# wyhuai/DDNM

Measured on AMD Instinct MI355X. Metric: restored images/sec @256×256, 100 DDIM steps, 4×SR; 1/2/4/8 GPU, higher is better.
Workload: dtype f32 (3x3 convolutions: fp32 operands carried as hi + lo fp16 halves, three fp16 MFMA products per product, fp32 accumulate -- operand error 2^-22, measured closer to fp64 than the fp32 MFMA kernel; everything else fp32); 1 GPU; celeba_hq.yml SVD sr_bicubic 4x, sigma_y=0, eta=0.85, T_sampling=100, batch_size=8 per GPU (BASELINE configs[1]); global_batch=8, image=3x256x256, parallelism=dp1 (image sharding)

## Files before the change

ddnm_amd/_lib.py:

```python
import ctypes
import os
from ctypes import POINTER, Structure, c_char_p, c_float, c_int32, c_int64, c_uint8, c_uint32, c_void_p

_HERE = os.path.dirname(os.path.abspath(__file__))
LIB_PATH = os.path.join(_HERE, "libddnm_hip.so")

c_f32p = c_void_p


class ConvDesc(Structure):
    _fields_ = [
        ("src0", c_void_p), ("src1", c_void_p), ("weight", c_void_p), ("bias", c_void_p),
        ("badd", c_void_p), ("res", c_void_p), ("gn_scale", c_void_p), ("gn_shift", c_void_p),
        ("out", c_void_p),
        ("B", c_int32), ("Hin", c_int32), ("Win", c_int32),
        ("C0", c_int32), ("C1", c_int32), ("Cout", c_int32),
        ("ksize", c_int32), ("stride", c_int32), ("pad", c_int32),
        ("Ho", c_int32), ("Wo", c_int32),
        ("ups", c_int32), ("gn_silu", c_int32), ("out_nchw", c_int32),
        ("badd_stride", c_int32), ("tile", c_int32),
        ("workspace", c_void_p), ("workspace_floats", c_int64),
        ("res_ups", c_int32), ("src_f16", c_int32),
        ("stats_out", c_void_p),
        ("skip0", c_void_p), ("skip1", c_void_p), ("skip_weight", c_void_p),
# ... 61 lines not shown
    "ddnm_hq_project_f32": (c_int32, [c_void_p, c_void_p, c_void_p, c_void_p, c_int64, c_float, c_void_p]),
    "ddnm_copy_rect_f32": (c_int32, [c_void_p, c_int32, c_int32, c_int32, c_int32, c_void_p, c_int32, c_int32, c_int32,
                                     c_int32, c_int32, c_int32, c_int32, c_void_p]),
    "ddnm_hq_sample_f32": (c_int32, [c_void_p, c_void_p, c_void_p, c_void_p, c_void_p, c_int64, c_float, c_float, c_float,
                                     c_float, c_void_p]),
    "ddnm_patchify_f32": (c_int32, [c_void_p, c_void_p, c_int32, c_int32, c_int32, c_int32, c_void_p]),
    "ddnm_im2col3x3_f16": (c_int32, [c_void_p, c_void_p, c_void_p, c_void_p, c_void_p, c_int32, c_int32, c_int32, c_int32,
                                     c_int32, c_int32, c_void_p]),
    "ddnm_gn_apply_f16": (c_int32, [c_void_p, c_void_p, c_void_p, c_void_p, c_void_p, c_int32, c_int32, c_int32, c_int32,
                                    c_int32, c_void_p]),
    "ddnm_gn_finalize_tiles_f32": (c_int32, [c_void_p, c_int32, c_int32, c_void_p, c_int32, c_int32, c_void_p, c_void_p,
                                             c_int32, c_int32, c_int32, c_float, c_void_p, c_void_p, c_void_p, c_int32,
                                             c_void_p, c_void_p]),
    "ddnm_gn_finalize_tiles_amax_f32": (c_int32, [c_void_p, c_int32, c_int32, c_void_p, c_int32, c_int32, c_void_p, c_void_p,
                                                  c_int32, c_int32, c_int32, c_float, c_void_p, c_void_p, c_void_p, c_int32,
                                                  c_void_p, c_void_p, c_void_p]),
    "ddnm_amax_bound_f32": (c_int32, [c_void_p, c_int64, c_int32, c_void_p, c_int64, c_int32, c_void_p, c_int32, c_void_p]),
    "ddnm_conv3x3_f16_f32": (c_int32, [POINTER(ConvDesc), c_void_p]),
    "ddnm_conv3x3_f16_supported": (c_int32, [POINTER(ConvDesc)]),
    "ddnm_conv3x3_f16_workspace_floats": (c_int64, [POINTER(ConvDesc)]),
    "ddnm_conv3x3_f16_stats_tiles": (c_int32, [POINTER(ConvDesc)]),
    "ddnm_conv3x3_s16_f32": (c_int32, [POINTER(ConvDesc), c_void_p]),
    "ddnm_conv3x3_s16_supported": (c_int32, [POINTER(ConvDesc)]),
    "ddnm_conv3x3_s16_persistent": (c_int32, [POINTER(ConvDesc)]),
    "ddnm_conv3x3_s16_ups_subpixel_supported": (c_int32, [POINTER(ConvDesc)]),
    "ddnm_conv3x3_s16_workspace_floats": (c_int64, [POINTER(ConvDesc)]),
    "ddnm_conv3x3_s16_stats_tiles": (c_int32, [POINTER(ConvDesc)]),
    "ddnm_conv3x3_s16_act_scale": (c_float, []),
    "ddnm_conv_gather_s16_f32": (c_int32, [POINTER(ConvDesc), c_void_p]),
    "ddnm_conv_gather_s16_supported": (c_int32, [POINTER(ConvDesc)]),
    "ddnm_conv_gather_s16_workspace_floats": (c_int64, [POINTER(ConvDesc)]),
    "ddnm_conv_gather_s16_stats_tiles": (c_int32, [POINTER(ConvDesc)]),
    "ddnm_conv_gather_s16_gemm1x1": (c_int32, [POINTER(ConvDesc)]),
    "ddnm_conv16": (c_int32, [POINTER(Conv16Desc), c_void_p]),
    "ddnm_conv16_supported": (c_int32, [POINTER(Conv16Desc)]),
    "ddnm_conv16_fuses_fin": (c_int32, [POINTER(Conv16Desc)]),
    "ddnm_conv16_workspace_floats": (c_int64, [POINTER(Conv16Desc)]),
    "ddnm_conv16_stats_tiles": (c_int32, [POINTER(Conv16Desc)]),
    "ddnm_gn_apply_h16": (c_int32, [c_void_p, c_void_p, c_void_p, c_void_p, c_void_p, c_int32, c_int32, c_int32, c_int32,
                                    c_int32, c_int32, c_int32, c_void_p]),
    "ddnm_im2col3x3_h16": (c_int32, [c_void_p, c_void_p, c_void_p, c_void_p, c_void_p, c_int32, c_int32, c_int32, c_int32,
                                     c_int32, c_int32, c_void_p]),
    "ddnm_nchw_to_nhwc_h16": (c_int32, [c_void_p, c_void_p, c_int32, c_int32, c_int32, c_int32, c_void_p]),
    "ddnm_gn_stats_h16": (c_int32, [c_void_p, c_void_p, c_int32, c_int32, c_int32, c_int32, c_void_p]),
    "ddnm_attn16_d64": (c_int32, [c_void_p, c_void_p, c_int32, c_int32, c_int32, c_void_p]),
    "ddnm_conv1x1_f16_f32": (c_int32, [POINTER(ConvDesc), c_void_p]),
    "ddnm_conv1x1_f16_supported": (c_int32, [POINTER(ConvDesc)]),
    "ddnm_conv1x1_f16_workspace_floats": (c_int64, [POINTER(ConvDesc)]),
    "ddnm_conv1x1_f16_stats_tiles": (c_int32, [POINTER(ConvDesc)]),
    "ddnm_gn_stats_f32": (c_int32, [c_void_p, c_void_p, c_int32, c_int32, c_int32, c_int32, c_int32, c_void_p,
                                    c_int32, c_void_p]),
    "ddnm_gn_nchunk": (c_int32, [c_int32, c_int32]),
    "ddnm_gn_finalize_f32": (c_int32, [c_void_p, c_int32, c_void_p, c_void_p, c_int32, c_int32, c_int32, c_int32,
                                       c_float, c_void_p, c_void_p, c_void_p, c_int32, c_void_p, c_void_p]),
    "ddnm_bgemm_f32": (c_int32, [POINTER(GemmDesc), c_void_p]),
    "ddnm_gn_bwd_f32": (c_int32, [c_void_p, c_void_p, c_int32, c_void_p, c_void_p, c_void_p, c_int32, c_void_p, c_int32,
                                  c_int32, c_int32, c_int32, c_int32, c_int32, c_void_p, c_int32, c_void_p, c_void_p,
                                  c_void_p]),
    "ddnm_gn_bwd_nchunk": (c_int32, [c_int32, c_int32]),
    "ddnm_gn_bwd_h16": (c_int32, [c_void_p, c_void_p, c_int32, c_void_p, c_void_p, c_void_p, c_int32, c_void_p, c_int32,
                                  c_int32, c_int32, c_int32, c_int32, c_int32, c_void_p, c_int32, c_void_p, c_void_p,
                                  c_void_p]),
    "ddnm_pool_tokens_h16": (c_int32, [c_void_p, c_void_p, c_void_p, c_void_p, c_void_p, c_int32, c_int32, c_int32,
                                       c_void_p]),
    "ddnm_pool_tokens_bwd_h16": (c_int32, [c_void_p, c_void_p, c_int32, c_int32, c_int32, c_void_p]),
    "ddnm_attn16_d64_lse": (c_int32, [c_void_p, c_void_p, c_void_p, c_int32, c_int32, c_int32, c_void_p]),
# ... 165 lines not shown
```

ddnm_amd/build.py:

```python
import hashlib
import os
import shutil
import subprocess
import sys

HERE = os.path.dirname(os.path.abspath(__file__))
CSRC = os.path.join(HERE, "csrc")
LIB = os.path.join(HERE, "libddnm_hip.so")
STAMP = os.path.join(HERE, ".libddnm_hip.stamp")
OBJ = os.path.join(HERE, "_obj")
SOURCES = ["conv_igemm_f32.hip", "conv_igemm_f16.hip", "conv_s16_persist.hip", "conv_s16_subpixel.hip", "conv_gather_s16.hip", "conv1x1_s16.hip", "conv_small_f32.hip", "conv1x1_f16.hip", "conv16.hip", "act16.hip", "attn16.hip", "attn_d512.hip", "attn16_bwd.hip", "gemm_f32.hip", "groupnorm.hip", "misc.hip", "ddnm_step.hip", "fwht.hip", "backward.hip", "metrics.hip"]
FLAGS = ["--offload-arch=gfx950", "-O3", "-std=c++17", "-fPIC", "-shared", "-Wall", "-Wno-unused-function"]


def _hipcc():
    for c in (os.environ.get("HIPCC"), shutil.which("hipcc"), "/opt/rocm/bin/hipcc"):
        if c and os.path.exists(c):
            return c
    raise RuntimeError("hipcc not found (set HIPCC)")


def _digest():
    h = hashlib.sha256()
    for f in sorted(os.listdir(CSRC)) + ["../../include/ddnm_hip.h"]:
        with open(os.path.join(CSRC, f), "rb") as fh:
            h.update(f.encode() + fh.read())
    h.update(" ".join(FLAGS).encode())
    return h.hexdigest()


LAST_BUILD = {"compiled": False}


def build(force=False, verbose=False):
    dig = _digest()
    LAST_BUILD["compiled"] = False
    if not force and os.path.exists(LIB) and os.path.exists(STAMP) and open(STAMP).read() == dig:
        return LIB
    LAST_BUILD["compiled"] = True
    tmp = LIB + f".tmp{os.getpid()}"
    os.makedirs(OBJ, exist_ok=True)
    hh = hashlib.sha256()
    for f in sorted(os.listdir(CSRC)) + ["../../include/ddnm_hip.h"]:
        if f.endswith(".h"):
# ... 54 lines not shown
```

ddnm_amd/csrc/conv1x1_s16.hip:

```cpp
#include "s16_tile.h"

constexpr int G1_KS = 2;
constexpr int G1_BM = 64, G1_BN = 64;
constexpr int G1_AR = G1_BM / 32;
constexpr int G1_BR = G1_BN / 32;
constexpr int G1_NWG = 3;
constexpr int G1_WSUB = G1_BN * 128;
constexpr int G1_ASUB = G1_BM * S16_LDH;
constexpr int G1_REQ_A = G1_KS * (G1_AR + 2);
constexpr int G1_REQ_W = G1_KS * G1_BR;
constexpr int G1_WAIT = 3 * G1_REQ_A + 2 * G1_REQ_W;
constexpr int G1_MAX_CIN = 1024;
constexpr int G1_ROUTE_MAX_CIN = 512;
static_assert(G1_WAIT < 64, "vmcnt counts to 63");

__device__ __forceinline__ void g1_tile_stats(float p0, float p1, float p2, float p3, int rows, float& s, float& q) {
#pragma clang fp contract(off)
    if (rows >= 4) {
        s = ((p0 + p1) + p2) + p3;
        q = ((p0 * p0 + p1 * p1) + p2 * p2) + p3 * p3;
    } else if (rows == 3) {
        s = ((p0 + p3) + p1) + p2;
        q = (__builtin_fmaf(p3, p3, p0 * p0) + p1 * p1) + p2 * p2;
    } else if (rows == 2) {
        s = (p0 + p2) + (p1 + p3);
        q = __builtin_fmaf(p2, p2, p0 * p0) + __builtin_fmaf(p3, p3, p1 * p1);
    } else {
        s = ((p0 + p1) + p2) + p3;
        q = __builtin_fmaf(p3, p3, __builtin_fmaf(p2, p2, __builtin_fmaf(p1, p1, p0 * p0)));
    }
}

__global__ __launch_bounds__(256) void conv1x1_s16_kernel(const ConvArgs p, const int stats_px) {
    __shared__ __attribute__((aligned(1024))) char lds_all[G1_NWG * G1_KS * G1_WSUB + G1_KS * G1_ASUB * 2];
    char* const Bs = lds_all;
    _Float16* const As = reinterpret_cast<_Float16*>(lds_all + G1_NWG * G1_KS * G1_WSUB);

    const ddnm_conv_desc& d = p.d;
    const int tid = threadIdx.x, lane = tid & 63, wave = tid >> 6;
    const int wm = wave >> 1, wn = wave & 1;
    const int tile_id = xcd_swizzle(blockIdx.x, gridDim.x);
    const int n_tile = tile_id % p.n_tiles, m_tile = tile_id / p.n_tiles;
    const int hw = d.Ho * d.Wo;
    const int img = m_tile / (hw / G1_BM);
    const unsigned pix0 = (unsigned)m_tile * G1_BM;
    float ascale, inv_ascale;
    s16_operand_scale(d.gn_scale == nullptr ? d.amax_in : nullptr, img, false, ascale, inv_ascale);

    const int lrow = lane >> 3, lpiece = lane & 7;
    const int wswz = S16_W_SWZ(wave, lrow);
    const unsigned w_rowlen = (unsigned)p.Cin * 4u;
    const int cout_pad = (d.Cout + 127) / 128 * 128;
    const __amdgpu_buffer_rsrc_t r_w = __builtin_amdgcn_make_buffer_rsrc(
        const_cast<void*>(reinterpret_cast<const void*>(d.weight)), 0, (unsigned)cout_pad * w_rowlen, 0x00020000);
    const unsigned w_voff = S16_W_LANE(n_tile * G1_BN + wave * 8 + lrow, w_rowlen, lpiece, wswz);
    const int nchunks = p.Cin / S16_KCH;
    const int nsteps = (nchunks + G1_KS - 1) / G1_KS;
    auto chunk_of = [&](int s, int sub) { const int c = s * G1_KS + sub; return c < nchunks ? c : nchunks - 1; };
    auto issue_w = [&](int s, int grp) {
#pragma unroll
        for (int sub = 0; sub < G1_KS; ++sub)
            s16_w_request<G1_BR, 4>(r_w, Bs + (grp * G1_KS + sub) * G1_WSUB + wave * 1024, w_voff, (unsigned)chunk_of(s, sub) * S16_KCH * 4u,
                                    w_rowlen);
    };
// ... 127 lines not shown
    }
    if (ksplit == 1) {
        float add = 0.f;
        if (d.bias) add = bias;
        if (d.badd) add += badd;
#pragma unroll
        for (int r = 0; r < 16; ++r) v[r] = acc[0][0][r] * epi + add + rv[r];
    } else if (d.stats_out) {
        float add = 0.f;
        if (d.bias) add = add + bias;
        if (d.badd) add = add + badd;
#pragma unroll
        for (int r = 0; r < 16; ++r) {
            v[r] = add + total[r] * epi;
            if (res) v[r] = v[r] + rv[r];
        }
    } else {
#pragma unroll
        for (int r = 0; r < 16; ++r) {
            v[r] = total[r] * epi;
            if (d.bias) v[r] = v[r] + bias;
            if (d.badd) v[r] = v[r] + badd;
            if (res) v[r] = v[r] + rv[r];
        }
    }
#pragma unroll
    for (int r = 0; r < 16; ++r) out[o[r]] = v[r];
    if (stats_px == 4) {
        const unsigned t0 = (pix0 + wm * 32 + rsel) >> 2;
        const int rows = 256 / (d.Cout >> 2);
#pragma unroll
        for (int q = 0; q < 4; ++q) {
            float cs, cq;
            g1_tile_stats(v[q * 4], v[q * 4 + 1], v[q * 4 + 2], v[q * 4 + 3], rows, cs, cq);
            float2* const st = reinterpret_cast<float2*>(d.stats_out + ((size_t)(t0 + 2 * q) * d.Cout + n) * 2);
            *st = make_float2(cs, cq);
        }
    } else if (stats_px == G1_BM) {
        float cs = 0.f, cq = 0.f;
#pragma unroll
        for (int r = 0; r < 16; ++r) {
            cs += v[r];
            cq = __builtin_fmaf(v[r], v[r], cq);
        }
        cs += __shfl_xor(cs, 32);
        cq += __shfl_xor(cq, 32);
        float* const lds = reinterpret_cast<float*>(As);
        __syncthreads();
        if (lane < 32) {
            lds[(wm * G1_BN + wn * 32 + lane) * 2 + 0] = cs;
            lds[(wm * G1_BN + wn * 32 + lane) * 2 + 1] = cq;
        }
        __syncthreads();
        if (tid < G1_BN * 2) {
            const int c = tid >> 1, which = tid & 1;
            d.stats_out[((size_t)m_tile * d.Cout + n_tile * G1_BN + c) * 2 + which] = lds[c * 2 + which] + lds[(G1_BN + c) * 2 + which];
        }
    }
}

int conv1x1_s16_stats_px(const ddnm_conv_desc* d, int plan_ksplit, int plan_bm) {
    if (!d->stats_out) return 0;
    if (plan_ksplit > 1) {
        const int tpi = splitk_stats_tiles(d);
        return tpi > 0 && d->Ho * d->Wo == 4 * tpi ? 4 : -1;
    }
    return plan_bm == G1_BM ? G1_BM : -1;
}

bool conv1x1_s16_routes(const ddnm_conv_desc* d, int plan_ksplit, int plan_bm) {
    const int hw = d->Ho * d->Wo, Cin = d->C0 + d->C1;
    if (d->ksize != 1 || d->stride != 1 || d->pad != 0 || d->ups || d->res_ups || d->out_nchw || d->skip0) return false;
    if (d->Ho != d->Hin || d->Wo != d->Win || hw % G1_BM || d->Cout % G1_BN) return false;
    if (d->C0 <= 0 || d->C0 % S16_KCH || d->C1 % S16_KCH || Cin > G1_MAX_CIN) return false;
    if (conv1x1_s16_stats_px(d, plan_ksplit, plan_bm) < 0) return false;
    if (d->flags & DDNM_CONV_GEMM1X1) return true;
    return Cin <= G1_ROUTE_MAX_CIN;
}

int conv1x1_s16_launch(const ddnm_conv_desc* d, int plan_ksplit, int plan_bm, int run_ksplit, hipStream_t s) {
    const ConvArgs p = conv_args(*d, G1_BM, d->Cout / G1_BN, 32, 5, 0, 1, run_ksplit);
    DDNM_LAUNCH(conv1x1_s16_kernel, dim3(p.m_tiles * p.n_tiles), dim3(256), 0, s, p, conv1x1_s16_stats_px(d, plan_ksplit, plan_bm));
    return 0;
}
```

ddnm_amd/csrc/conv_common.h:

```cpp
#pragma once
#include "common.h"

struct ConvArgs {
    ddnm_conv_desc d;
    int Cin, ntaps, Hs, Ws;
    int m_tiles, n_tiles;
    int tiles_x;
    int TW, TW_log2;
    int ksplit;
    float* ws;
};

static inline bool conv_operand_offsets_fit(const ddnm_conv_desc* d) {
    const int64_t px = (int64_t)d->B * (d->ups ? d->Hin / 2 : d->Hin) * (d->ups ? d->Win / 2 : d->Win);
    const int64_t cmax = d->C0 > d->C1 ? d->C0 : d->C1;
    return px * cmax * (d->src_f16 ? 2 : 4) < (int64_t)1 << 31;
}
static inline bool conv_sizes_addressable(const ddnm_conv_desc* d) {
    const int64_t lim = (int64_t)1 << 31;
    const int64_t out_el = (int64_t)d->B * d->Ho * d->Wo * d->Cout;
    const int64_t cout_pad = ((int64_t)d->Cout + 127) / 128 * 128;
    const int64_t w_b = cout_pad * d->ksize * d->ksize * ((int64_t)d->C0 + d->C1) * 4;
    const int64_t sk_el = (int64_t)d->B * d->Ho * d->Wo * (d->SC0 > d->SC1 ? d->SC0 : d->SC1);
    return out_el < lim && conv_operand_offsets_fit(d) && w_b < lim && sk_el < lim;
}

bool conv3x3_s16_persist_eligible(const ConvArgs& p);
int conv3x3_s16_persist_launch(const ConvArgs& p, hipStream_t s);
bool conv3x3_s16_ups_subpixel_ok(const ddnm_conv_desc* d);
int conv3x3_s16_ups_subpixel_run(const ddnm_conv_desc* d, hipStream_t s);
bool conv1x1_s16_routes(const ddnm_conv_desc* d, int plan_ksplit, int plan_bm);
int conv1x1_s16_launch(const ddnm_conv_desc* d, int plan_ksplit, int plan_bm, int run_ksplit, hipStream_t s);
int conv_persist_grid_cus();

struct TileMap {
    int img, ty0, tx0, th_unused, TW, TW_log2, flat_base, Wo;
    bool two_d;
    __device__ __forceinline__ void pixel(int r, int& oy, int& ox) const {
        if (two_d) {
            oy = ty0 + (r >> TW_log2);
            ox = tx0 + (r & (TW - 1));
        } else {
            const int pix = flat_base + r;
            oy = pix / Wo;
            ox = pix - oy * Wo;
        }
    }
};

template <int BM>
__device__ __forceinline__ TileMap make_tilemap(const ConvArgs& p, int m_tile) {
    TileMap t;
    const int HWo = p.d.Ho * p.d.Wo;
    const int per_img = HWo / BM;
    t.img = m_tile / per_img;
    const int t_in_img = m_tile - t.img * per_img;
    t.TW = p.TW;
    t.TW_log2 = p.TW_log2;
    t.Wo = p.d.Wo;
    t.two_d = p.tiles_x != 0;
    if (t.two_d) {
        const int ty = t_in_img / p.tiles_x, tx = t_in_img - ty * p.tiles_x;
        t.ty0 = ty * (BM >> p.TW_log2);
        t.tx0 = tx << p.TW_log2;
        t.flat_base = 0;
// ... 236 lines not shown
            if (d.res) {
                if (d.res_ups) {
                    const int oy = p2 / d.Wo, ox = p2 - oy * d.Wo;
                    v = v + *reinterpret_cast<const f32x4*>(d.res + (((size_t)b * (d.Ho >> 1) + (oy >> 1)) * (d.Wo >> 1) + (ox >> 1)) * d.Cout + n);
                } else {
                    v = v + reinterpret_cast<const f32x4*>(d.res)[i];
                }
            }
            reinterpret_cast<f32x4*>(d.out)[i] = v;
            s += v;
            ss += v * v;
        }
    }
    red[0][tid] = s;
    red[1][tid] = ss;
    __syncthreads();
    if (tid < c4n) {
        for (int r = 1; r < rows; ++r) { s += red[0][r * c4n + tid]; ss += red[1][r * c4n + tid]; }
        float* o = d.stats_out + ((size_t)blockIdx.x * d.Cout + tid * 4) * 2;
        f32x4 lo = {s.x, ss.x, s.y, ss.y}, hi = {s.z, ss.z, s.w, ss.w};
        reinterpret_cast<f32x4*>(o)[0] = lo;
        reinterpret_cast<f32x4*>(o)[1] = hi;
    }
}

static inline int splitk_stats_tiles(const ddnm_conv_desc* d) {
    const int hw = d->Ho * d->Wo;
    if (d->out_nchw || d->Cout % 4 || d->Cout > 1024 || hw % 4) return 0;
    int tpi = hw / 4 < 128 ? hw / 4 : 128;
    while (tpi > 1 && hw % tpi) --tpi;
    return tpi;
}

static inline int launch_splitk_reduce(const ConvArgs& p, hipStream_t s) {
    const ddnm_conv_desc& d = p.d;
    if (d.stats_out) {
        const int tpi = splitk_stats_tiles(&d);
        if (tpi <= 0) return DDNM_E_SHAPE;
        DDNM_LAUNCH(conv_splitk_reduce_stats_kernel, dim3(d.B * tpi), dim3(256), 0, s, p, tpi);
        return 0;
    }
    const size_t total4 = (size_t)d.B * d.Ho * d.Wo * d.Cout / 4;
    const unsigned g = (unsigned)((total4 + 255) / 256 < 2048 ? (total4 + 255) / 256 : 2048);
    DDNM_LAUNCH(conv_splitk_reduce_kernel, dim3(g), dim3(256), 0, s, p, total4);
    return 0;
}

static inline int conv_check_desc(const ddnm_conv_desc* d, int no_src1 = DDNM_E_BADARG) {
    if (!d || !d->src0 || !d->weight || !d->out) return DDNM_E_BADARG;
    if (d->B <= 0 || d->Cout <= 0 || d->Ho <= 0 || d->Wo <= 0) return DDNM_E_BADARG;
    if (!conv_sizes_addressable(d)) return DDNM_E_SHAPE;
    if (d->C1 > 0 && !d->src1) return no_src1;
    return 0;
}

static inline int conv_check_gn_ups(const ddnm_conv_desc* d) {
    if (d->gn_scale && !d->gn_shift) return DDNM_E_BADARG;
    if (d->ups && ((d->Hin | d->Win) & 1)) return DDNM_E_SHAPE;
    if (d->res_ups && ((d->Ho | d->Wo) & 1)) return DDNM_E_SHAPE;
    return 0;
}

static inline int64_t conv_slab_floats(const ddnm_conv_desc* d, int ksplit) {
    return ksplit > 1 ? (int64_t)ksplit * d->B * d->Ho * d->Wo * d->Cout : 0;
}

// ... 27 lines not shown
```

ddnm_amd/csrc/conv_gather_s16.hip:

```cpp
#include "s16_tile.h"

constexpr int GS_KC = S16_KCH, GS_LDH = S16_LDH;

template <int WM, int WN, int MT, int NT>
__global__ __launch_bounds__(256) void conv_gather_s16_kernel(const ConvArgs p) {
    constexpr int BM = WM * MT * 32, BN = WN * NT * 32;
    constexpr int AR = BM / 32, BR = BN / 32;
    constexpr int NWB = 3;
    constexpr int WTILE = BN * 128;
    __shared__ __attribute__((aligned(1024))) char lds_all[NWB * WTILE + BM * GS_LDH * 2];
    char* const Bs = lds_all;
    _Float16* const As = reinterpret_cast<_Float16*>(lds_all + NWB * WTILE);

    const ddnm_conv_desc& d = p.d;
    const int tid = threadIdx.x, lane = tid & 63, wave = tid >> 6;
    const int wm = wave / WN, wn = wave % WN;
    const int tile_id = xcd_swizzle(blockIdx.x, gridDim.x);
    const int n_tile = tile_id % p.n_tiles, m_tile = tile_id / p.n_tiles;
    const int slice = blockIdx.y;
    const TileMap tm = make_tilemap<BM>(p, m_tile);
    const int img = tm.img;
    float ascale, inv_ascale;
    s16_operand_scale(d.gn_scale == nullptr ? d.amax_in : nullptr, img, false, ascale, inv_ascale);

// ... 135 lines not shown
    if (d->Cout % 4 == 0 && tiles < 192) {
        ks = (int)((512 + tiles - 1) / tiles);
        if (ks > nchunks) ks = nchunks;
        if (ks > 16) ks = 16;
        if (ks < 1) ks = 1;
    }
    pl->ksplit = ks;
    return true;
}

extern "C" int ddnm_conv_gather_s16_supported(const ddnm_conv_desc* d) {
    PlanGS pl;
    return d && plan_gs(d, &pl) ? 1 : 0;
}

extern "C" int64_t ddnm_conv_gather_s16_workspace_floats(const ddnm_conv_desc* d) {
    PlanGS pl;
    if (!d || !plan_gs(d, &pl)) return DDNM_E_SHAPE;
    return conv_slab_floats(d, pl.ksplit);
}

extern "C" int ddnm_conv_gather_s16_stats_tiles(const ddnm_conv_desc* d) {
    PlanGS pl;
    if (!d || !plan_gs(d, &pl)) return DDNM_E_SHAPE;
    return conv_stats_tiles(d, pl.ksplit, pl.BM);
}

extern "C" int ddnm_conv_gather_s16_gemm1x1(const ddnm_conv_desc* d) {
    PlanGS pl;
    if (!d || !plan_gs(d, &pl)) return DDNM_E_SHAPE;
    return !(d->flags & DDNM_CONV_ONE_TILE) && conv1x1_s16_routes(d, pl.ksplit, pl.BM) ? 1 : 0;
}

extern "C" int ddnm_conv_gather_s16_f32(const ddnm_conv_desc* d, void* stream) {
    if (int e = conv_check_desc(d)) return e;
    if (!(d->acc_scale > 0.f)) return DDNM_E_BADARG;
    if (!d->gn_scale && !d->amax_in) return DDNM_E_BADARG;
    if (int e = conv_check_gn_ups(d)) return e;
    PlanGS pl;
    if (!plan_gs(d, &pl)) return DDNM_E_SHAPE;
    const int plan_ksplit = pl.ksplit;
    if ((pl.ksplit = conv_run_ksplit(d, pl.ksplit)) < 0) return pl.ksplit;
    if (!(d->flags & DDNM_CONV_ONE_TILE) && conv1x1_s16_routes(d, plan_ksplit, pl.BM))
        return conv1x1_s16_launch(d, plan_ksplit, pl.BM, pl.ksplit, (hipStream_t)stream);
    const ConvArgs p = conv_args(*d, pl.BM, d->Cout / pl.BN, 32, 5, 0, d->ksize * d->ksize, pl.ksplit);
    const dim3 grid(p.m_tiles * p.n_tiles, pl.ksplit);
    hipStream_t s = (hipStream_t)stream;
    if (pl.tile == 1) { DDNM_LAUNCH((conv_gather_s16_kernel<2, 2, 2, 2>), grid, dim3(256), 0, s, p); }
    else { DDNM_LAUNCH((conv_gather_s16_kernel<2, 2, 1, 1>), grid, dim3(256), 0, s, p); }
    if (pl.ksplit > 1) return launch_splitk_reduce(p, s);
    return 0;
}
```

ddnm_amd/csrc/s16_tile.h:

```cpp
#pragma once
#include "conv_common.h"

typedef unsigned u32x4 __attribute__((ext_vector_type(4)));

constexpr int S16_WM = 4, S16_WN = 2, S16_MT = 2, S16_NT = 2;
constexpr int S16_NTHREADS = S16_WM * S16_WN * 64, S16_BN = S16_WN * S16_NT * 32;
constexpr int S16_KCH = 32;
constexpr int S16_LDH = 72;
constexpr int S16_MAXH = 340, S16_HWD = 34;
constexpr int S16_HCOLS = 8;
constexpr int S16_HRPP = S16_NTHREADS / S16_HCOLS;
constexpr int S16_HR = (S16_MAXH + S16_HRPP - 1) / S16_HRPP, S16_HSPLIT = (S16_HR + 1) / 2;
constexpr int S16_BR = S16_BN / (S16_NTHREADS / 8);
constexpr int S16_NWB = 3;
constexpr int S16_WTILE = S16_BN * 128;
constexpr int S16_HBYTES = 2 * S16_MAXH * S16_LDH * 2;
constexpr int S16_NOUT = S16_MT * S16_NT * 16;
constexpr unsigned S16_OOB = 0x80000000u;

#define S16_W_SWZ(wave, lrow) ((((wave) & 1) << 2) | ((lrow) >> 1))
#define S16_W_LANE(row, rowlen, lpiece, wswz) ((unsigned)(row) * (rowlen) + (unsigned)(((lpiece) ^ (wswz)) * 16))
#define S16_B_FRAG(row0, lane) ((((row0) + ((lane) & 31)) * 128) + (((((lane) >> 5) ^ ((((lane) & 31) >> 1) & 7))) << 4))
template <int BR, int NWAVES>
__device__ __forceinline__ void s16_w_request(const __amdgpu_buffer_rsrc_t& r_w, char* dst, const unsigned& w_lane, unsigned so,
// ... 60 lines not shown
        const float add = addv[j];
#pragma unroll
        for (int i = 0; i < MT; ++i)
#pragma unroll
            for (int r = 0; r < 16; ++r) {
                const int k = (i * NT + j) * 16 + r;
                float v = acc[i][j][r] * epi + add;
                if constexpr (RES != S16_RES_NONE) v = v + (RES == S16_RES_TILE ? outv[k] : 0.f);
                outv[k] = v;
                cs[j] += v;
                cq[j] = __builtin_fmaf(v, v, cq[j]);
                acc[i][j][r] = 0.f;
            }
        cs[j] += __shfl_xor(cs[j], 32);
        cq[j] += __shfl_xor(cq[j], 32);
    }
    if (lane < 32) {
#pragma unroll
        for (int j = 0; j < NT; ++j) {
            const int c = (wn * NT + j) * 32 + lane;
            stat_lds[(wm * BN + c) * 2 + 0] = cs[j];
            stat_lds[(wm * BN + c) * 2 + 1] = cq[j];
        }
    }
}
__device__ __forceinline__ void s16_store_stats(const float* stat_lds, int tid, const __amdgpu_buffer_rsrc_t r_stats, unsigned st_lane,
                                                unsigned st_soff) {
    const int c = (tid >> 1) & (S16_BN - 1), which = tid & 1;
    float a = 0.f;
#pragma unroll
    for (int w = 0; w < S16_WM; ++w) a += stat_lds[(w * S16_BN + c) * 2 + which];
    __builtin_amdgcn_raw_buffer_store_b32(__float_as_uint(a), r_stats, st_lane, st_soff, 0);
}
```

include/ddnm_hip.h:

```cpp
#ifndef DDNM_HIP_H
#define DDNM_HIP_H

#include <stdint.h>

#ifdef __cplusplus
extern "C" {
#endif

#define DDNM_E_BADARG (-1)
#define DDNM_E_SHAPE (-2)

int ddnm_version(void);
const char* ddnm_build_digest(void);
int ddnm_sizeof(int which);
const char* ddnm_error_string(int code);

typedef struct ddnm_conv_desc {
    const float* src0;
    const float* src1;
    const float* weight;
    const float* bias;
    const float* badd;
    const float* res;
    const float* gn_scale;
// ... 27 lines not shown

#define DDNM_CONV_ONE_TILE 1
#define DDNM_CONV_UPS_SUBPIXEL 2
#define DDNM_CONV_GEMM1X1 4
#define DDNM_AMAX_N 32

int ddnm_conv2d_f32(const ddnm_conv_desc* d, void* stream);
int ddnm_conv2d_f32_tile_n(const ddnm_conv_desc* d);
int64_t ddnm_conv2d_f32_workspace_floats(const ddnm_conv_desc* d);
int ddnm_conv2d_f32_stats_tiles(const ddnm_conv_desc* d);
int ddnm_conv2d_f32_fuses_skip(const ddnm_conv_desc* d);

int ddnm_conv3x3_small_cout_f32(const ddnm_conv_desc* d, void* stream);
int ddnm_conv3x3_small_cout_f32_supported(const ddnm_conv_desc* d);

int ddnm_conv3x3_f16_f32(const ddnm_conv_desc* d, void* stream);
int ddnm_conv3x3_f16_supported(const ddnm_conv_desc* d);
int64_t ddnm_conv3x3_f16_workspace_floats(const ddnm_conv_desc* d);
int ddnm_conv3x3_f16_stats_tiles(const ddnm_conv_desc* d);

int ddnm_conv3x3_s16_f32(const ddnm_conv_desc* d, void* stream);
int ddnm_conv3x3_s16_supported(const ddnm_conv_desc* d);
int ddnm_conv3x3_s16_persistent(const ddnm_conv_desc* d);
int64_t ddnm_conv3x3_s16_workspace_floats(const ddnm_conv_desc* d);
int ddnm_conv3x3_s16_stats_tiles(const ddnm_conv_desc* d);
int ddnm_conv3x3_s16_ups_subpixel_supported(const ddnm_conv_desc* d);
float ddnm_conv3x3_s16_act_scale(void);

int ddnm_conv_gather_s16_f32(const ddnm_conv_desc* d, void* stream);
int ddnm_conv_gather_s16_supported(const ddnm_conv_desc* d);
int64_t ddnm_conv_gather_s16_workspace_floats(const ddnm_conv_desc* d);
int ddnm_conv_gather_s16_stats_tiles(const ddnm_conv_desc* d);
int ddnm_conv_gather_s16_gemm1x1(const ddnm_conv_desc* d);

int ddnm_conv1x1_f16_f32(const ddnm_conv_desc* d, void* stream);
int ddnm_conv1x1_f16_supported(const ddnm_conv_desc* d);
int64_t ddnm_conv1x1_f16_workspace_floats(const ddnm_conv_desc* d);
int ddnm_conv1x1_f16_stats_tiles(const ddnm_conv_desc* d);

typedef struct ddnm_conv16_desc {
    const void* src;
    const void* weight;
    const float* bias;
    const void* res;
    const void* skip0;
    const void* skip1;
    const void* skip_weight;
    void* out;
    float* stats_out;
    float* workspace;
    int64_t workspace_floats;
    int32_t B, H, W;
    int32_t Cin, Cout;
    int32_t ksize;
    int32_t ups, res_ups;
    int32_t SC0, SC1;
    const void* src1;
    const float* gn_scale;
    const float* gn_shift;
    int32_t C0;
    int32_t gn_silu;
    int32_t out_nchw_f32;
    int32_t reserved;
    const float* fin_gamma;
    const float* fin_beta;
    const float* fin_film;
// ... 282 lines not shown
```

Baseline: 6.433 images/sec.

## Add intra-workgroup split-K kernel for 8x8 3x3 convolutions

Adds a new 3x3 convolution kernel for 8x8 spatial layers in which the split-K slices run as waves inside one workgroup. Each wave stages its own halo and weight tile in LDS, and the partial sums are reduced through LDS slabs in the epilogue. This replaces the multi-block split-K launch plus separate reduce kernel for the low-resolution UNet levels, removing a workspace round-trip and a kernel launch. It needs a large LDS footprint per workgroup, and the fp32 reduction order changes. The quad-stats helper is moved to a shared header for reuse.

```diff
diff --git a/ddnm_amd/_lib.py b/ddnm_amd/_lib.py
--- a/ddnm_amd/_lib.py
+++ b/ddnm_amd/_lib.py
@@ -117,6 +117,7 @@
     "ddnm_conv_gather_s16_workspace_floats": (c_int64, [POINTER(ConvDesc)]),
     "ddnm_conv_gather_s16_stats_tiles": (c_int32, [POINTER(ConvDesc)]),
     "ddnm_conv_gather_s16_gemm1x1": (c_int32, [POINTER(ConvDesc)]),
+    "ddnm_conv_gather_s16_wslice": (c_int32, [POINTER(ConvDesc)]),
     "ddnm_conv16": (c_int32, [POINTER(Conv16Desc), c_void_p]),
     "ddnm_conv16_supported": (c_int32, [POINTER(Conv16Desc)]),
     "ddnm_conv16_fuses_fin": (c_int32, [POINTER(Conv16Desc)]),
diff --git a/ddnm_amd/build.py b/ddnm_amd/build.py
--- a/ddnm_amd/build.py
+++ b/ddnm_amd/build.py
@@ -9,7 +9,7 @@
 LIB = os.path.join(HERE, "libddnm_hip.so")
 STAMP = os.path.join(HERE, ".libddnm_hip.stamp")
 OBJ = os.path.join(HERE, "_obj")
-SOURCES = ["conv_igemm_f32.hip", "conv_igemm_f16.hip", "conv_s16_persist.hip", "conv_s16_subpixel.hip", "conv_gather_s16.hip", "conv1x1_s16.hip", "conv_small_f32.hip", "conv1x1_f16.hip", "conv16.hip", "act16.hip", "attn16.hip", "attn_d512.hip", "attn16_bwd.hip", "gemm_f32.hip", "groupnorm.hip", "misc.hip", "ddnm_step.hip", "fwht.hip", "backward.hip", "metrics.hip"]
+SOURCES = ["conv_igemm_f32.hip", "conv_igemm_f16.hip", "conv_s16_persist.hip", "conv_s16_subpixel.hip", "conv_gather_s16.hip", "conv1x1_s16.hip", "conv_s16_wslice.hip", "conv_small_f32.hip", "conv1x1_f16.hip", "conv16.hip", "act16.hip", "attn16.hip", "attn_d512.hip", "attn16_bwd.hip", "gemm_f32.hip", "groupnorm.hip", "misc.hip", "ddnm_step.hip", "fwht.hip", "backward.hip", "metrics.hip"]
 FLAGS = ["--offload-arch=gfx950", "-O3", "-std=c++17", "-fPIC", "-shared", "-Wall", "-Wno-unused-function"]
 
 
diff --git a/ddnm_amd/csrc/conv1x1_s16.hip b/ddnm_amd/csrc/conv1x1_s16.hip
--- a/ddnm_amd/csrc/conv1x1_s16.hip
+++ b/ddnm_amd/csrc/conv1x1_s16.hip
@@ -13,23 +13,6 @@
 constexpr int G1_MAX_CIN = 1024;
 constexpr int G1_ROUTE_MAX_CIN = 512;
 static_assert(G1_WAIT < 64, "vmcnt counts to 63");
-
-__device__ __forceinline__ void g1_tile_stats(float p0, float p1, float p2, float p3, int rows, float& s, float& q) {
-#pragma clang fp contract(off)
-    if (rows >= 4) {
-        s = ((p0 + p1) + p2) + p3;
-        q = ((p0 * p0 + p1 * p1) + p2 * p2) + p3 * p3;
-    } else if (rows == 3) {
-        s = ((p0 + p3) + p1) + p2;
-        q = (__builtin_fmaf(p3, p3, p0 * p0) + p1 * p1) + p2 * p2;
-    } else if (rows == 2) {
-        s = (p0 + p2) + (p1 + p3);
-        q = __builtin_fmaf(p2, p2, p0 * p0) + __builtin_fmaf(p3, p3, p1 * p1);
-    } else {
-        s = ((p0 + p1) + p2) + p3;
-        q = __builtin_fmaf(p3, p3, __builtin_fmaf(p2, p2, __builtin_fmaf(p1, p1, p0 * p0)));
-    }
-}
 
 __global__ __launch_bounds__(256) void conv1x1_s16_kernel(const ConvArgs p, const int stats_px) {
     __shared__ __attribute__((aligned(1024))) char lds_all[G1_NWG * G1_KS * G1_WSUB + G1_KS * G1_ASUB * 2];
@@ -223,7 +206,7 @@
 #pragma unroll
         for (int q = 0; q < 4; ++q) {
             float cs, cq;
-            g1_tile_stats(v[q * 4], v[q * 4 + 1], v[q * 4 + 2], v[q * 4 + 3], rows, cs, cq);
+            s16_quad_stats(v[q * 4], v[q * 4 + 1], v[q * 4 + 2], v[q * 4 + 3], rows, cs, cq);
             float2* const st = reinterpret_cast<float2*>(d.stats_out + ((size_t)(t0 + 2 * q) * d.Cout + n) * 2);
             *st = make_float2(cs, cq);
         }
@@ -252,10 +235,7 @@
 
 int conv1x1_s16_stats_px(const ddnm_conv_desc* d, int plan_ksplit, int plan_bm) {
     if (!d->stats_out) return 0;
-    if (plan_ksplit > 1) {
-        const int tpi = splitk_stats_tiles(d);
-        return tpi > 0 && d->Ho * d->Wo == 4 * tpi ? 4 : -1;
-    }
+    if (plan_ksplit > 1) return splitk_stats_are_quads(d) ? 4 : -1;
     return plan_bm == G1_BM ? G1_BM : -1;
 }
 
diff --git a/ddnm_amd/csrc/conv_common.h b/ddnm_amd/csrc/conv_common.h
--- a/ddnm_amd/csrc/conv_common.h
+++ b/ddnm_amd/csrc/conv_common.h
@@ -31,6 +31,8 @@
 int conv3x3_s16_ups_subpixel_run(const ddnm_conv_desc* d, hipStream_t s);
 bool conv1x1_s16_routes(const ddnm_conv_desc* d, int plan_ksplit, int plan_bm);
 int conv1x1_s16_launch(const ddnm_conv_desc* d, int plan_ksplit, int plan_bm, int run_ksplit, hipStream_t s);
+bool conv3x3_s16_wslice_routes(const ddnm_conv_desc* d, int plan_ksplit, int plan_bm);
+int conv3x3_s16_wslice_launch(const ddnm_conv_desc* d, int ksplit, hipStream_t s);
 int conv_persist_grid_cus();
 
 struct TileMap {
@@ -333,6 +335,11 @@
     return tpi;
 }
 
+static inline bool splitk_stats_are_quads(const ddnm_conv_desc* d) {
+    const int tpi = splitk_stats_tiles(d);
+    return tpi > 0 && d->Ho * d->Wo == 4 * tpi;
+}
+
 static inline int launch_splitk_reduce(const ConvArgs& p, hipStream_t s) {
     const ddnm_conv_desc& d = p.d;
     if (d.stats_out) {
diff --git a/ddnm_amd/csrc/conv_gather_s16.hip b/ddnm_amd/csrc/conv_gather_s16.hip
--- a/ddnm_amd/csrc/conv_gather_s16.hip
+++ b/ddnm_amd/csrc/conv_gather_s16.hip
@@ -191,6 +191,12 @@
     return !(d->flags & DDNM_CONV_ONE_TILE) && conv1x1_s16_routes(d, pl.ksplit, pl.BM) ? 1 : 0;
 }
 
+extern "C" int ddnm_conv_gather_s16_wslice(const ddnm_conv_desc* d) {
+    PlanGS pl;
+    if (!d || !plan_gs(d, &pl)) return DDNM_E_SHAPE;
+    return !(d->flags & DDNM_CONV_ONE_TILE) && conv3x3_s16_wslice_routes(d, pl.ksplit, pl.BM) ? 1 : 0;
+}
+
 extern "C" int ddnm_conv_gather_s16_f32(const ddnm_conv_desc* d, void* stream) {
     if (int e = conv_check_desc(d)) return e;
     if (!(d->acc_scale > 0.f)) return DDNM_E_BADARG;
@@ -202,6 +208,8 @@
     if ((pl.ksplit = conv_run_ksplit(d, pl.ksplit)) < 0) return pl.ksplit;
     if (!(d->flags & DDNM_CONV_ONE_TILE) && conv1x1_s16_routes(d, plan_ksplit, pl.BM))
         return conv1x1_s16_launch(d, plan_ksplit, pl.BM, pl.ksplit, (hipStream_t)stream);
+    if (!(d->flags & DDNM_CONV_ONE_TILE) && pl.ksplit == plan_ksplit && conv3x3_s16_wslice_routes(d, plan_ksplit, pl.BM))
+        return conv3x3_s16_wslice_launch(d, plan_ksplit, (hipStream_t)stream);
     const ConvArgs p = conv_args(*d, pl.BM, d->Cout / pl.BN, 32, 5, 0, d->ksize * d->ksize, pl.ksplit);
     const dim3 grid(p.m_tiles * p.n_tiles, pl.ksplit);
     hipStream_t s = (hipStream_t)stream;
diff --git a/ddnm_amd/csrc/conv_s16_wslice.hip b/ddnm_amd/csrc/conv_s16_wslice.hip
--- /dev/null
+++ b/ddnm_amd/csrc/conv_s16_wslice.hip
@@ -0,0 +1,216 @@
+#include "s16_tile.h"
+
+constexpr int WS_WAVES = 8, WS_NTHREADS = WS_WAVES * 64;
+constexpr int WS_BM = 64, WS_BN = 32;
+constexpr int WS_HW = 10, WS_HROWS = WS_HW * WS_HW;
+constexpr int WS_HSLOTS = (WS_HROWS + 7) / 8;
+constexpr int WS_HALO = WS_HROWS * S16_LDH;
+constexpr int WS_WTILE = WS_BN * 128;
+constexpr int WS_BR = WS_BN / 8;
+constexpr int WS_NB = 3;
+constexpr int WS_SP = WS_BN + 8;
+constexpr int WS_SLAB = WS_BM * WS_SP;
+constexpr int WS_LDS_MAIN = WS_WAVES * (WS_HALO * 2 + WS_WTILE), WS_LDS_RED = WS_WAVES * WS_SLAB * 4;
+constexpr int WS_LDS = WS_LDS_MAIN > WS_LDS_RED ? WS_LDS_MAIN : WS_LDS_RED;
+static_assert(WS_LDS <= 160 * 1024, "LDS of one CU");
+
+__global__ __launch_bounds__(WS_NTHREADS) void conv_s16_wslice_kernel(const ConvArgs p) {
+    constexpr int MT = 2, NT = 1, BN = WS_BN, SP = WS_SP, SLAB = WS_SLAB;
+    __shared__ __attribute__((aligned(1024))) char lds_all[WS_LDS];
+
+    const ddnm_conv_desc& d = p.d;
+    const int tid = threadIdx.x, lane = tid & 63;
+    const int wave = __builtin_amdgcn_readfirstlane(tid >> 6);
+    const int tile_id = xcd_swizzle(blockIdx.x, gridDim.x);
+    const int n_tile = tile_id % p.n_tiles, m_tile = tile_id / p.n_tiles;
+    const int per_img = p.tiles_x * (d.Ho >> 3);
+    const int img = m_tile / per_img, t_in_img = m_tile - img * per_img;
+    const int ty0 = (t_in_img / p.tiles_x) << 3, tx0 = (t_in_img % p.tiles_x) << 3;
+    float ascale, inv_ascale;
+    s16_operand_scale(d.gn_scale == nullptr ? d.amax_in : nullptr, img, false, ascale, inv_ascale);
+
+    const int lrow = lane >> 3, lpiece = lane & 7;
+    const unsigned w_rowlen = 9u * (unsigned)p.Cin * 4u;
+    const int cout_pad = (d.Cout + 127) / 128 * 128;
+    const __amdgpu_buffer_rsrc_t r_w = __builtin_amdgcn_make_buffer_rsrc(
+        const_cast<void*>(reinterpret_cast<const void*>(d.weight)), 0, (unsigned)cout_pad * w_rowlen, 0x00020000);
+    unsigned w_voff[2];
+#pragma unroll
+    for (int o = 0; o < 2; ++o) w_voff[o] = S16_W_LANE(n_tile * BN + lrow, w_rowlen, lpiece, (o << 2) | (lrow >> 1));
+    auto load_b = [&](int chunk, int tap, u32x4 (&b)[WS_BR]) {
+        const unsigned so = ((unsigned)tap * (unsigned)p.Cin + (unsigned)chunk * S16_KCH) * 4u;
+#pragma unroll
+        for (int j = 0; j < WS_BR; ++j)
+            b[j] = __builtin_amdgcn_raw_buffer_load_b128(r_w, w_voff[j & 1], so + (unsigned)j * 8u * w_rowlen, 0);
+    };
+    char* const wtile = lds_all + WS_WAVES * WS_HALO * 2 + wave * WS_WTILE;
+    auto stage_b = [&](const u32x4 (&b)[WS_BR]) {
+#pragma unroll
+        for (int j = 0; j < WS_BR; ++j) *reinterpret_cast<u32x4*>(wtile + j * 1024 + lane * 16) = b[j];
+    };
+    const int b_frag = S16_B_FRAG(0, lane);
+
+    const bool has_gn = d.gn_scale != nullptr;
+    const int c4 = lane & 7, hr0 = lane >> 3;
+    const __amdgpu_buffer_rsrc_t r_s0 = __builtin_amdgcn_make_buffer_rsrc(
+        const_cast<float*>(d.src0), 0, (unsigned)d.B * d.Hin * d.Win * d.C0 * 4u, 0x00020000);
+    const __amdgpu_buffer_rsrc_t r_s1 = __builtin_amdgcn_make_buffer_rsrc(
+        const_cast<float*>(d.C1 > 0 ? d.src1 : d.src0), 0, (unsigned)d.B * d.Hin * d.Win * (d.C1 > 0 ? d.C1 : d.C0) * 4u, 0x00020000);
+    int hpix[WS_HSLOTS];
+#pragma unroll
+    for (int i = 0; i < WS_HSLOTS; ++i) {
+        const int r = hr0 + 8 * i;
+        const int hy = (r * 205) >> 11, hx = r - hy * WS_HW;
+        const int iy = ty0 + hy - 1, ix = tx0 + hx - 1;
+        const bool ok = r < WS_HROWS && (unsigned)iy < (unsigned)d.Hin && (unsigned)ix < (unsigned)d.Win;
+        hpix[i] = ok ? (img * d.Hin + iy) * d.Win + ix : -1;
+    }
+    struct Halo {
+        f32x4 v[WS_HSLOTS], gsc, gsh;
+    };
+    auto prefetch_a = [&](int chunk, Halo& h) {
+        const int cb = chunk * S16_KCH;
+        const bool first = cb < d.C0;
+        const unsigned cs = first ? d.C0 : d.C1, coff = first ? cb : cb - d.C0;
+        const __amdgpu_buffer_rsrc_t r_s = first ? r_s0 : r_s1;
+#pragma unroll
+        for (int i = 0; i < WS_HSLOTS; ++i) {
+            const unsigned vo = hpix[i] >= 0 ? ((unsigned)hpix[i] * cs + c4 * 4) * 4u : S16_OOB;
+            h.v[i] = __builtin_bit_cast(f32x4, __builtin_amdgcn_raw_buffer_load_b128(r_s, vo, coff * 4u, 0));
+        }
+        if (has_gn) {
+            h.gsc = *reinterpret_cast<const f32x4*>(d.gn_scale + (size_t)img * p.Cin + cb + c4 * 4);
+            h.gsh = *reinterpret_cast<const f32x4*>(d.gn_shift + (size_t)img * p.Cin + cb + c4 * 4);
+        }
+    };
+    _Float16* const halo = reinterpret_cast<_Float16*>(lds_all) + wave * WS_HALO;
+    auto stage_a = [&](const Halo& h) {
+#pragma unroll
+        for (int i = 0; i < WS_HSLOTS; ++i) {
+            f32x4 v = h.v[i];
+            if (has_gn && hpix[i] >= 0) v = gn_act(v, h.gsc, h.gsh, d.gn_silu);
+            if (hr0 + 8 * i < WS_HROWS) split_store(&halo[(hr0 + 8 * i) * S16_LDH + c4 * 4], v, ascale);
+        }
+    };
+
+    f32x16 acc[MT][NT];
+#pragma unroll
+    for (int i = 0; i < MT; ++i)
+#pragma unroll
+        for (int j = 0; j < NT; ++j)
+#pragma unroll
+            for (int r = 0; r < 16; ++r) acc[i][j][r] = 0.f;
+
+    const int nchunks = p.Cin / S16_KCH, ksplit = p.ksplit;
+    const int c_begin = wave < ksplit ? (int)((long)nchunks * wave / ksplit) : 0;
+    const int c_end = wave < ksplit ? (int)((long)nchunks * (wave + 1) / ksplit) : 0;
+    const _Float16* const a_frag = halo + (((lane & 31) >> 3) * WS_HW + (lane & 7)) * S16_LDH + (lane >> 5) * 8;
+
+    if (c_begin < c_end) {
+        Halo h;
+        u32x4 b[WS_NB][WS_BR];
+        prefetch_a(c_begin, h);
+        load_b(c_begin, 0, b[0]);
+        load_b(c_begin, 1, b[1]);
+        for (int c = c_begin; c < c_end; ++c) {
+            stage_a(h);
+            const bool more = c + 1 < c_end;
+            const int cn = more ? c + 1 : c;
+            if (more) prefetch_a(cn, h);
+            __builtin_amdgcn_sched_barrier(0);
+#pragma unroll
+            for (int tap = 0; tap < 9; ++tap) {
+                const int t2 = tap + 2 < 9 ? tap + 2 : tap + 2 - 9;
+                load_b(tap + 2 < 9 ? c : cn, t2, b[(tap + 2) % WS_NB]);
+                stage_b(b[tap % WS_NB]);
+                __builtin_amdgcn_wave_barrier();
+                __builtin_amdgcn_sched_barrier(0);
+                int a_rows[MT];
+#pragma unroll
+                for (int i = 0; i < MT; ++i) a_rows[i] = i * 4 * WS_HW * S16_LDH;
+                s16_mfma_tile<MT, NT>(acc, a_frag, a_rows, ((tap / 3) * WS_HW + tap % 3) * S16_LDH, wtile, b_frag);
+                __builtin_amdgcn_sched_barrier(0);
+            }
+        }
+    }
+
+    float* const slabs = reinterpret_cast<float*>(lds_all);
+    __syncthreads();
+    if (wave < ksplit) {
+        float* const mine = slabs + wave * SLAB;
+        const int rsel = 4 * (lane >> 5);
+#pragma unroll
+        for (int i = 0; i < MT; ++i)
+#pragma unroll
+            for (int j = 0; j < NT; ++j)
+#pragma unroll
+                for (int r = 0; r < 16; ++r)
+                    mine[(i * 32 + (r & 3) + 8 * (r >> 2) + rsel) * SP + j * 32 + (lane & 31)] = acc[i][j][r];
+    }
+    __syncthreads();
+
+    const float epi = d.acc_scale * inv_ascale;
+    const int nl = tid % BN, q0 = tid / BN;
+    const int n = n_tile * BN + nl;
+    const float bias = d.bias ? d.bias[n] : 0.f, badd = d.badd ? d.badd[(size_t)img * d.badd_stride + n] : 0.f;
+    const float* __restrict__ res = d.res;
+    float* __restrict__ out = d.out;
+    const int rows = 256 / (d.Cout >> 2);
+    unsigned o[NT][4], pixq[NT];
+    float rv[NT][4];
+#pragma unroll
+    for (int k = 0; k < NT; ++k) {
+        const int m0 = (q0 + (WS_NTHREADS / BN) * k) * 4;
+        const unsigned pix0 = pixq[k] = (unsigned)((img * d.Ho + ty0 + (m0 >> 3)) * d.Wo + tx0 + (m0 & 7));
+#pragma unroll
+        for (int e = 0; e < 4; ++e) {
+            o[k][e] = (pix0 + e) * (unsigned)d.Cout + (unsigned)n;
+            rv[k][e] = res ? res[o[k][e]] : 0.f;
+        }
+    }
+#pragma unroll
+    for (int k = 0; k < NT; ++k) {
+        const int m0 = (q0 + (WS_NTHREADS / BN) * k) * 4;
+        float v[4];
+#pragma unroll
+        for (int e = 0; e < 4; ++e) {
+            float total = 0.f;
+#pragma unroll
+            for (int s = 0; s < WS_WAVES; ++s)
+                if (s < ksplit) total = total + slabs[s * SLAB + (m0 + e) * SP + nl];
+            if (d.stats_out) {
+                float add = 0.f;
+                if (d.bias) add = add + bias;
+                if (d.badd) add = add + badd;
+                v[e] = add + total * epi;
+                if (res) v[e] = v[e] + rv[k][e];
+            } else {
+                v[e] = total * epi;
+                if (d.bias) v[e] = v[e] + bias;
+                if (d.badd) v[e] = v[e] + badd;
+                if (res) v[e] = v[e] + rv[k][e];
+            }
+            out[o[k][e]] = v[e];
+        }
+        if (d.stats_out) {
+            float cs, cq;
+            s16_quad_stats(v[0], v[1], v[2], v[3], rows, cs, cq);
+            *reinterpret_cast<float2*>(d.stats_out + ((size_t)(pixq[k] >> 2) * d.Cout + n) * 2) = make_float2(cs, cq);
+        }
+    }
+}
+
+bool conv3x3_s16_wslice_routes(const ddnm_conv_desc* d, int plan_ksplit, int plan_bm) {
+    if (d->ksize != 3 || d->stride != 1 || d->pad != 1 || d->ups || d->res_ups || d->out_nchw || d->skip0) return false;
+    if (d->Ho != 8 || d->Wo != 8 || d->Hin != 8 || d->Win != 8) return false;
+    if (d->C0 <= 0 || d->C0 % S16_KCH || d->C1 % S16_KCH || d->Cout % 64) return false;
+    if (plan_ksplit < 2 || plan_ksplit > WS_WAVES || plan_bm != WS_BM) return false;
+    if (d->stats_out && !splitk_stats_are_quads(d)) return false;
+    return true;
+}
+
+int conv3x3_s16_wslice_launch(const ddnm_conv_desc* d, int ksplit, hipStream_t s) {
+    const ConvArgs p = conv_args(*d, WS_BM, d->Cout / WS_BN, 8, 3, d->Wo / 8, 9, ksplit);
+    DDNM_LAUNCH(conv_s16_wslice_kernel, dim3(p.m_tiles * p.n_tiles), dim3(WS_NTHREADS), 0, s, p);
+    return 0;
+}
diff --git a/ddnm_amd/csrc/s16_tile.h b/ddnm_amd/csrc/s16_tile.h
--- a/ddnm_amd/csrc/s16_tile.h
+++ b/ddnm_amd/csrc/s16_tile.h
@@ -116,3 +116,20 @@
     for (int w = 0; w < S16_WM; ++w) a += stat_lds[(w * S16_BN + c) * 2 + which];
     __builtin_amdgcn_raw_buffer_store_b32(__float_as_uint(a), r_stats, st_lane, st_soff, 0);
 }
+
+__device__ __forceinline__ void s16_quad_stats(float p0, float p1, float p2, float p3, int rows, float& s, float& q) {
+#pragma clang fp contract(off)
+    if (rows >= 4) {
+        s = ((p0 + p1) + p2) + p3;
+        q = ((p0 * p0 + p1 * p1) + p2 * p2) + p3 * p3;
+    } else if (rows == 3) {
+        s = ((p0 + p3) + p1) + p2;
+        q = (__builtin_fmaf(p3, p3, p0 * p0) + p1 * p1) + p2 * p2;
+    } else if (rows == 2) {
+        s = (p0 + p2) + (p1 + p3);
+        q = __builtin_fmaf(p2, p2, p0 * p0) + __builtin_fmaf(p3, p3, p1 * p1);
+    } else {
+        s = ((p0 + p1) + p2) + p3;
+        q = __builtin_fmaf(p3, p3, __builtin_fmaf(p2, p2, __builtin_fmaf(p1, p1, p0 * p0)));
+    }
+}
diff --git a/include/ddnm_hip.h b/include/ddnm_hip.h
--- a/include/ddnm_hip.h
+++ b/include/ddnm_hip.h
@@ -83,6 +83,7 @@
 int64_t ddnm_conv_gather_s16_workspace_floats(const ddnm_conv_desc* d);
 int ddnm_conv_gather_s16_stats_tiles(const ddnm_conv_desc* d);
 int ddnm_conv_gather_s16_gemm1x1(const ddnm_conv_desc* d);
+int ddnm_conv_gather_s16_wslice(const ddnm_conv_desc* d);
 
 int ddnm_conv1x1_f16_f32(const ddnm_conv_desc* d, void* stream);
 int ddnm_conv1x1_f16_supported(const ddnm_conv_desc* d);
```

New measurement: 6.534 images/sec (median of 6 runs). +1.6%, better.
